# eglrp/fSGM

Hardware: AMD Instinct MI355X
Metric: aggregated cost-volume voxel-paths/s (HxWxDx8 paths), KITTI 1242x375 D=128 (higher is better)
Workload: dtype u8

## Files before the change

### fsgm_amd/csrc/epi_band.hip

```cpp
#include "epi_kernels.h"
#include "fsgm_device.h"
#include "epi_step.h"
#include <type_traits>
#include <stdlib.h>

namespace fsgm {

#ifndef FSGM_BAND_PF
#define FSGM_BAND_PF 2
#endif
#ifndef FSGM_BAND_PF2
#define FSGM_BAND_PF2 1
#endif
#ifndef FSGM_BAND_PF4
#define FSGM_BAND_PF4 3
#endif
#ifndef FSGM_BAND_PFE
#define FSGM_BAND_PFE 4
#endif
#ifndef FSGM_BAND_PFE2
#define FSGM_BAND_PFE2 2
#endif
#ifndef FSGM_BAND_R16
#define FSGM_BAND_R16 1
#endif
#ifndef FSGM_BAND_Y16
#define FSGM_BAND_Y16 0
#endif
#ifndef FSGM_BAND_RECLDS
#define FSGM_BAND_RECLDS 1
#endif
#ifndef FSGM_BAND_SLACK
#define FSGM_BAND_SLACK 32
#endif
#ifndef FSGM_BAND_WAVES
#define FSGM_BAND_WAVES 8
#endif
#ifndef FSGM_BAND_MINW
#define FSGM_BAND_MINW 4
#endif

__device__ __forceinline__ uint32_t pack_hi_bits(const uint32_t (&R)[8]) {
    constexpr uint32_t SEL_HI = 0x07030501u;
    const uint32_t h0 = __builtin_amdgcn_perm(R[1], R[0], SEL_HI), h1 = __builtin_amdgcn_perm(R[3], R[2], SEL_HI);
    const uint32_t h2 = __builtin_amdgcn_perm(R[5], R[4], SEL_HI), h3 = __builtin_amdgcn_perm(R[7], R[6], SEL_HI);
    return h0 | (h1 << 1) | (h2 << 2) | (h3 << 3);
}
__device__ __forceinline__ void unpack_p9(const uint4 v, const uint32_t bits, uint32_t (&R)[8]) {
    const uint32_t w[4] = {v.x, v.y, v.z, v.w};
#pragma unroll
    for (int k = 0; k < 4; k++) {
        const uint32_t hk = (bits >> k) & 0x01010101u;
        R[2 * k] = __builtin_amdgcn_perm(hk, w[k], 0x06020400u);
        R[2 * k + 1] = __builtin_amdgcn_perm(hk, w[k], 0x07030501u);
    }
}

__device__ __forceinline__ void band_unpack_c(const uint4 w, uint32_t (&C)[8]) {
    C[0] = __builtin_amdgcn_perm(w.z, w.x, 0x0C040C00u);
    C[1] = __builtin_amdgcn_perm(w.z, w.x, 0x0C050C01u);
    C[2] = __builtin_amdgcn_perm(w.z, w.x, 0x0C060C02u);
    C[3] = __builtin_amdgcn_perm(w.z, w.x, 0x0C070C03u);
    C[4] = __builtin_amdgcn_perm(w.w, w.y, 0x0C040C00u);
    C[5] = __builtin_amdgcn_perm(w.w, w.y, 0x0C050C01u);
    C[6] = __builtin_amdgcn_perm(w.w, w.y, 0x0C060C02u);
    C[7] = __builtin_amdgcn_perm(w.w, w.y, 0x0C070C03u);
}
template <int LPP, bool MASKED, bool OUT_N>
__device__ __forceinline__ void step_x(uint32_t (&S)[8], const uint32_t (&C)[8], uint32_t (&O)[8], const uint32_t P1pk,
                                       const uint32_t P2pk, const uint32_t kx, const uint32_t K0, const LaneSel sel,
                                       const bool start) {
    uint32_t N[8], YB[8];
    const uint32_t LT = __builtin_amdgcn_perm(S[7], (uint32_t)__builtin_amdgcn_mov_dpp((int)S[7], DPP_ROW_SHR1, 0xF, 0xF, true), sel.lo);
    const uint32_t RT = __builtin_amdgcn_perm((uint32_t)__builtin_amdgcn_mov_dpp((int)S[0], DPP_ROW_SHL1, 0xF, 0xF, true), S[0], sel.hi);
#pragma unroll
    for (int i = 0; i < 8; i++) {
        YB[i] = pk_max3(S[i] + P1pk, i ? S[i - 1] : LT, i < 7 ? S[i + 1] : RT);
        asm("v_xad_u32 %0, %1, %2, %3" : "=v"(N[i]) : "v"(YB[i]), "s"(kx), "v"(C[i]));
    }
    const uint32_t mm = pk_min(pk_min3(N[0], N[1], N[2]), pk_min3(N[3], N[4], pk_min3(N[5], N[6], N[7])));
    uint32_t mx = group_min_u32<LPP>(min_halves(mm));
    if (MASKED && start) mx = K0;
    const uint32_t p2m = __umul24(mx, 0x10001u) + P2pk;
#pragma unroll
    for (int i = 0; i < 8; i++) {
        S[i] = pk_subs(p2m, N[i]);
        O[i] = OUT_N ? N[i] : YB[i];
    }
}

template <int LPP, int NT>
__device__ __forceinline__ uint2 band_nb_entry(const uint32_t d) {
    constexpr uint32_t D = LPP * 16;
    const uint32_t lo = d > 0 ? srow_index<NT>(0, d - 1) * 2u : 0u, hi = d + 1 < D ? srow_index<NT>(0, d + 1) * 2u : 0u;
    return make_uint2(lo | (hi << 16), (d > 0 ? 0x0000FFFFu : 0u) | (d + 1 < D ? 0xFFFF0000u : 0u));
}
template <uint32_t X>
__device__ __forceinline__ uint32_t sconst() { uint32_t r; asm("s_mov_b32 %0, %1" : "=s"(r) : "i"(X)); return r; }

template <int LPP, int NT, bool STAGE>
__device__ __forceinline__ void band_wta_record(const uint32_t (&ST)[8], uint32_t* sRow, const uint2* sNb, int tid, int j,
                                                bool ok, uint8_t* recb, uint8_t* s0b, uint32_t pix,
                                                uint2* stg_rec, uint16_t* stg_s0) {
    srow_store<NT>(sRow, tid, ST);
    const uint32_t IDX[8] = {sconst<0x80000u>(), sconst<0x90001u>(), sconst<0xA0002u>(), sconst<0xB0003u>(),
                             sconst<0xC0004u>(), sconst<0xD0005u>(), sconst<0xE0006u>(), sconst<0xF0007u>()};
    uint32_t K[8];
#pragma unroll
    for (int i = 0; i < 8; i++) K[i] = (ST[i] << 4) | IDX[i];
    const uint32_t kmin = pk_min(pk_min3(K[0], K[1], K[2]), pk_min3(K[3], K[4], pk_min3(K[5], K[6], K[7])));
    const uint32_t k16 = min_halves(kmin);
    uint32_t key;
    asm("v_lshl_or_b32 %0, %1, 4, %2" : "=v"(key) : "v"(k16 & ~15u), "v"((k16 & 15u) | ((uint32_t)j << 4)));
    key = group_min_u32<LPP>(key);
    __builtin_amdgcn_wave_barrier();
    if (j == 0 && ok) {
        const uint2 nb = sNb[key & 0xFFu];
        const uint8_t* row = (const uint8_t*)sRow + tid * 16;
        u16x2 c;
        c[0] = *(const uint16_t*)(row + (nb.x & 0xFFFFu));
        c[1] = *(const uint16_t*)(row + (nb.x >> 16));
        const uint2 rec = make_uint2(__builtin_amdgcn_perm(0u, key, sconst<0x02010C00u>()),
                                     __builtin_bit_cast(uint32_t, c) & nb.y);
        if (STAGE) {
            *stg_rec = rec;
            *stg_s0 = (uint16_t)ST[0];
        } else {
            *(uint2*)(recb + pix * 8u) = rec;
            *(uint16_t*)(s0b + pix * 2u) = (uint16_t)ST[0];
        }
    }
}

template <int LPP, int MODE, int NWV, int PATHS, bool BITS, bool TAP, bool CHAIN>
__global__ __launch_bounds__(NWV * 64, FSGM_BAND_MINW) void band_kernel(BandArgs a) {
    constexpr bool UP = MODE != 0;
    constexpr bool P8 = PATHS == 8;
    constexpr int PXG = 64 / LPP;
    constexpr int R = NWV * PXG;
    constexpr int D = LPP * 16;
    constexpr int SKEW = P8 ? 2 : 1;
    constexpr int NST = P8 ? 3 : 1;
    constexpr int PF = P8 ? (MODE == 2 ? FSGM_BAND_PF2 : FSGM_BAND_PF) : FSGM_BAND_PF4;
    constexpr bool R16 = P8 && MODE == 0 && !CHAIN && FSGM_BAND_R16 != 0;
    constexpr int NSL = R16 ? 2 : NST;
    __shared__ uint2 sNb[MODE == 2 ? D : 1];
    __shared__ uint4 sR16[R16 ? 2 : 1][2][R16 ? (R + 1) * LPP : 1];
    __shared__ uint4 sSt[2][NSL][(R + 1) * LPP];
    __shared__ __attribute__((aligned(16))) uint32_t sRow[MODE == 2 ? NWV * 64 * 8 : 4];
    constexpr bool RECLDS = MODE == 2 && FSGM_BAND_RECLDS != 0 && LPP == 8;
    __shared__ uint2 sRec[RECLDS ? NWV * 64 : 1];
    __shared__ uint16_t sRs0[RECLDS ? NWV * 64 : 1];
    __shared__ uint32_t sTicket;

    const int tid = threadIdx.x, lane = tid & 63, wave = tid >> 6;
    const int g = lane / LPP, j = lane % LPP;
    const int r = wave * PXG + g;
    const int W = a.W, H = a.H, NP = W * H;
    int cband = 0;
    size_t f = blockIdx.x;
    if (CHAIN) {
        if (tid == 0) sTicket = atomicAdd(a.ticket, 1u);
        __syncthreads();
        const uint32_t t = __builtin_amdgcn_readfirstlane(sTicket);
        const uint32_t per = (uint32_t)a.group * (uint32_t)a.nbands, grp = t / per, rem = t - grp * per;
        const uint32_t fin = min((uint32_t)a.group, (uint32_t)a.frames - grp * (uint32_t)a.group);
        cband = (int)(rem / fin);
        f = (size_t)grp * a.group + rem % fin;
        if (cband >= a.nbands || f >= (size_t)a.frames) return;
    }
    constexpr uint32_t VB = (uint32_t)(SKEW * R + PF) * D;
    constexpr bool Y16 = BITS && FSGM_BAND_Y16 != 0;
    const uint8_t* __restrict__ Cf = a.C + f * a.c_frame_stride - VB;
    uint8_t* __restrict__ Yf = a.Y + f * a.y_frame_stride - VB;
    uint8_t* __restrict__ Bf = BITS ? (uint8_t*)(a.Yb + f * a.yb_frame_stride) - (Y16 ? VB : VB / 4) : nullptr;
    uint8_t* __restrict__ Ef = (uint8_t*)(a.edge + f * a.edge_frame_stride);
    const uint32_t tag = CHAIN ? a.tag : 0u;
    uint8_t* __restrict__ recb = MODE == 2 ? (uint8_t*)(a.rec + f * (size_t)NP) : nullptr;
    uint8_t* __restrict__ s0b = MODE == 2 ? (uint8_t*)(a.s0 + f * (size_t)NP) : nullptr;
    const uint32_t P1pk = (uint32_t)a.P1 * 0x10001u, P2 = (uint32_t)a.P2, P2pk = P2 * 0x10001u;
    const uint32_t KX = sconst<0x007F007Fu>(), K0 = 127u - (P2 + (uint32_t)a.P1);
    const uint32_t K1pk = (uint32_t)(PATHS * (a.P1 + a.P2) - (PATHS / 2) * 127) * 0x10001u;
    const uint4 startP = make_uint4(P2 * 0x01010101u, P2 * 0x01010101u, P2 * 0x01010101u, P2 * 0x01010101u);
    const uint32_t DS = sconst<(uint32_t)D>();
    const LaneSel sel = lane_sel<LPP>(j);
    const int elane = min(lane, NST * LPP - 1);

    if (MODE == 2 && tid < D) sNb[tid] = band_nb_entry<LPP, NWV * 64>((uint32_t)tid);

    auto pix_of = [&](int x, int y) -> int { const int p = y * W + x; return UP ? NP - 1 - p : p; };

    for (int yb = CHAIN ? cband * R : 0; yb < (CHAIN ? cband * R + 1 : H); yb += R) {
        const int Rp = min(R, H - yb);
        const int y = yb + r, yc = min(y, H - 1);
        const bool row_ok = r < Rp;
        const int nsteps = W + SKEW * (Rp - 1);
        const bool have_above = yb > 0, last_band = yb + R >= H;
        const bool loader = wave == 0 && lane < NST * LPP && have_above;
        const int r_lo = wave * PXG, r_hi = r_lo + PXG - 1;
        const int act_lo = SKEW * r_lo - (P8 ? 1 : 0), act_hi = W - 1 + SKEW * r_hi;
        const bool wave_rows = r_lo < Rp;
        const int pl_lo = SKEW * r_hi + 1, pl_hi = W - 2 + SKEW * r_lo;
        const bool wave_plain_rows = r_hi < Rp && yb + r_lo >= 1;

        auto vox_lin = [&](int x) -> uint32_t { return (uint32_t)pix_of(x, yc) * D + ((uint32_t)j * 16 + VB); };
        auto vox_off = [&](int u) -> uint32_t { return vox_lin(min(max(u - SKEW * r, 0), W - 1)); };
        uint32_t vpf = vox_lin(PF - 1 - SKEW * r);
        const uint32_t v_lo = vox_lin(UP ? W - 1 : 0), v_hi = vox_lin(UP ? 0 : W - 1);
        const uint32_t emap = (uint32_t)W * (NST * LPP) * 16u;
        const uint8_t* __restrict__ Ein = CHAIN ? Ef + (uint32_t)max(cband - 1, 0) * emap : Ef;
        uint8_t* __restrict__ Eout = CHAIN ? Ef + (uint32_t)cband * emap : Ef;
        auto edge_at = [&](int x) -> const uint8_t* { return Ein + ((uint32_t)min(max(x, 0), W - 1) * (NST * LPP) + (uint32_t)elane) * 16u; };
        bool gave_up = false;
        auto put_above = [&](const int par, const uint4 v) {
            if (R16 && elane / LPP == 2) {
                uint32_t S[8];
                unpack_p(v, S);
                sR16[par][0][elane % LPP] = make_uint4(S[0], S[1], S[2], S[3]);
                sR16[par][1][elane % LPP] = make_uint4(S[4], S[5], S[6], S[7]);
            } else {
                sSt[par][elane / LPP][elane % LPP] = v;
            }
        };
        auto fresh = [&](const uint4 v) -> bool { return (((v.x ^ tag) | (v.y ^ tag) | (v.z ^ tag) | (v.w ^ tag)) & 0x80808080u) == 0u; };
        auto eload = [&](const uint8_t* q) -> uint4 { return CHAIN ? edge_load((const uint4*)q) : load_nt(q); };
        auto settle = [&](uint4 v, const uint8_t* q, const bool mine) -> uint4 {
            if (CHAIN) {
                for (uint32_t spins = 0; !gave_up && !__all(!mine || fresh(v)); spins++) {
                    __builtin_amdgcn_s_sleep(8);
                    if (mine) v = edge_load((const uint4*)q);
                    if (spins > (1u << 18) || ((spins & 1023u) == 1023u && __hip_atomic_load(a.err, __ATOMIC_RELAXED, __HIP_MEMORY_SCOPE_AGENT) != 0u)) {
                        if (lane == 0) atomicOr(a.err, 1u);
                        gave_up = true;
                    }
                }
                v.x &= 0x7F7F7F7Fu; v.y &= 0x7F7F7F7Fu; v.z &= 0x7F7F7F7Fu; v.w &= 0x7F7F7F7Fu;
            }
            return v;
        };

        uint32_t FS[8];
#pragma unroll
        for (int i = 0; i < 8; i++) FS[i] = P2pk;
        uint4 hU = startP, hDp[2] = {startP, startP};
        if (P8 && have_above && wave == 0) {
            const bool mine = r == 0;
            const uint8_t* q0 = Ein + (uint32_t)(0 * LPP + j) * 16u;
            const uint8_t* q1 = Ein + (uint32_t)(1 * LPP + j) * 16u;
            const uint4 v0 = settle(mine ? eload(q0) : startP, q0, mine), v1 = settle(mine ? eload(q1) : startP, q1, mine);
            if (mine) { hU = v0; hDp[1] = v1; }
        }
        if (CHAIN && wave == 0 && have_above) {
            const uint8_t* q = edge_at(min(SKEW + FSGM_BAND_SLACK, W - 1));
            (void)settle(loader ? eload(q) : startP, q, loader);
        }
        if (wave == 0 && have_above) {
            const uint8_t* q = edge_at(SKEW - 1);
            const uint4 v = settle(loader ? eload(q) : startP, q, loader);
            if (loader) put_above(1, v);
        }
        constexpr int NR = MODE == 2 && P8 ? PF + 1 : PF;
        constexpr int UN = P8 && (NR & 1) ? 2 * NR : NR;
        uint4 ringC[NR], ringY[MODE == 2 ? NR : 1];
        constexpr int PFE = CHAIN ? (MODE == 2 ? FSGM_BAND_PFE2 : FSGM_BAND_PFE) : 1;
        uint4 ringE[PFE];
#pragma unroll
        for (int i = 0; i < PFE; i++) ringE[i] = startP;
        uint32_t ringB[MODE == 2 && BITS && !Y16 ? NR : 1];
        uint4 ringB4[MODE == 2 && Y16 ? NR : 1];
#pragma unroll
        for (int i = 0; i < PF; i++) {
            const uint32_t off = vox_off(i);
            ringC[i] = *(const uint4*)(Cf + off);
            if (MODE == 2) {
                ringY[i] = vol_load(Yf + off);
                if (Y16) ringB4[i] = vol_load(Bf + off);
                else if (BITS) ringB[i] = *(const uint32_t*)(Bf + (off >> 2));
            }
        }
        if (loader) {
#pragma unroll
            for (int i = 0; i < PFE; i++) ringE[i] = eload(edge_at(SKEW + i));
        }
        if constexpr (RECLDS) sRec[wave * 64 + lane] = make_uint2(0xFFFFFFFFu, 0xFFFFFFFFu);
        __syncthreads();

        auto do_step = [&](const int u, const int hp, const uint4 cw, const uint4 cy, const uint32_t cb, const uint4 cb4, auto edge_tag) {
            constexpr bool EDGE = decltype(edge_tag)::value;
            const int par = u & 1;
            const int x = u - SKEW * r;
            const bool inside = !EDGE || (row_ok && x >= 0 && x < W);
            const int xc = EDGE ? min(max(x, 0), W - 1) : x;
            uint4 nNow, nLo, nHi;
            if constexpr (R16) { nLo = sR16[par ^ 1][0][r * LPP + j]; nHi = sR16[par ^ 1][1][r * LPP + j]; }
            else nNow = sSt[par ^ 1][P8 ? 2 : 0][r * LPP + j];
            uint32_t CP[8], Y[8], YS[8], S[8];
            band_unpack_c(cw, CP);
            const bool top = EDGE && y == 0;
            {
                const bool st = EDGE && x <= 0;
                if (st) {
#pragma unroll
                    for (int i = 0; i < 8; i++) FS[i] = P2pk;
                }
                step_x<LPP, EDGE, MODE == 2>(FS, CP, YS, P1pk, P2pk, KX, K0, sel, st);
            }
            if (MODE == 2) {
                uint32_t E2[8];
                if (Y16) { E2[0] = cy.x; E2[1] = cy.y; E2[2] = cy.z; E2[3] = cy.w; E2[4] = cb4.x; E2[5] = cb4.y; E2[6] = cb4.z; E2[7] = cb4.w; }
                else if (BITS) unpack_p9(cy, cb, E2);
                else unpack_p(cy, E2);
#pragma unroll
                for (int i = 0; i < 8; i++) YS[i] -= E2[i];
            }
            __builtin_amdgcn_sched_barrier(0);
            uint4 newU, newD, newR;
            {
                unpack_p(P8 ? hU : nNow, S);
                if (top) {
#pragma unroll
                    for (int i = 0; i < 8; i++) S[i] = P2pk;
                }
                step_x<LPP, EDGE, MODE == 2>(S, CP, Y, P1pk, P2pk, KX, K0, sel, top);
                newU = pack_p(S);
                sSt[par][0][(r + 1) * LPP + j] = newU;
#pragma unroll
                for (int i = 0; i < 8; i++) YS[i] += MODE == 2 ? Y[i] + K1pk : Y[i];
            }
            __builtin_amdgcn_sched_barrier(0);
            if constexpr (P8) {
                {
                    const bool st = top || (EDGE && x <= 0);
                    unpack_p(hDp[hp], S);
                    if (st) {
#pragma unroll
                        for (int i = 0; i < 8; i++) S[i] = P2pk;
                    }
                    step_x<LPP, EDGE, MODE == 2>(S, CP, Y, P1pk, P2pk, KX, K0, sel, st);
                    newD = pack_p(S);
                    sSt[par][1][(r + 1) * LPP + j] = newD;
#pragma unroll
                    for (int i = 0; i < 8; i++) YS[i] += Y[i];
                    hDp[hp] = sSt[par ^ 1][1][r * LPP + j];
                    hU = sSt[par ^ 1][0][r * LPP + j];
                }
                __builtin_amdgcn_sched_barrier(0);
                {
                    const bool st = top || (EDGE && x >= W - 1);
                    if (R16) { S[0] = nLo.x; S[1] = nLo.y; S[2] = nLo.z; S[3] = nLo.w; S[4] = nHi.x; S[5] = nHi.y; S[6] = nHi.z; S[7] = nHi.w; }
                    else unpack_p(nNow, S);
                    if (st) {
#pragma unroll
                        for (int i = 0; i < 8; i++) S[i] = P2pk;
                    }
                    step_x<LPP, EDGE, MODE == 2>(S, CP, Y, P1pk, P2pk, KX, K0, sel, st);
                    if constexpr (R16) {
                        sR16[par][0][(r + 1) * LPP + j] = make_uint4(S[0], S[1], S[2], S[3]);
                        sR16[par][1][(r + 1) * LPP + j] = make_uint4(S[4], S[5], S[6], S[7]);
                        if (!last_band && r == R - 1) newR = pack_p(S);
                    } else {
                        newR = pack_p(S);
                        sSt[par][2][(r + 1) * LPP + j] = newR;
                    }
#pragma unroll
                    for (int i = 0; i < 8; i++) YS[i] += Y[i];
                }
            }
            if (!last_band && r == R - 1 && inside) {
                uint8_t* o = Eout + ((uint32_t)xc * (NST * LPP) + (uint32_t)j) * 16u;
                if (CHAIN) {
                    edge_store((uint4*)o, make_uint4(newU.x | tag, newU.y | tag, newU.z | tag, newU.w | tag));
                    if constexpr (P8) {
                        edge_store((uint4*)(o + LPP * 16), make_uint4(newD.x | tag, newD.y | tag, newD.z | tag, newD.w | tag));
                        edge_store((uint4*)(o + 2 * LPP * 16), make_uint4(newR.x | tag, newR.y | tag, newR.z | tag, newR.w | tag));
                    }
                } else {
                    *(uint4*)o = newU;
                    if constexpr (P8) { *(uint4*)(o + LPP * 16) = newD; *(uint4*)(o + 2 * LPP * 16) = newR; }
                }
            }
            if (MODE != 2) {
                if (inside) {
                    const uint32_t so = EDGE ? vox_lin(xc) : vpf;
                    constexpr int SB = EDGE ? 0 : PF * D;
                    if (Y16) {
                        vol_store(Yf + so - SB, make_uint4(YS[0], YS[1], YS[2], YS[3]));
                        vol_store(Bf + so - SB, make_uint4(YS[4], YS[5], YS[6], YS[7]));
                    } else {
                        vol_store(Yf + so - SB, pack_p(YS));
                        if (BITS) *(uint32_t*)(Bf + (so >> 2) - SB / 4) = pack_hi_bits(YS);
                    }
                }
            } else {
                uint32_t ST[8];
#pragma unroll
                for (int i = 0; i < 8; i++) ST[i] = (CP[i] << (P8 ? 2 : 1)) + YS[i];
                if constexpr (RECLDS)
                    band_wta_record<LPP, NWV * 64, true>(ST, sRow, sNb, tid, j, inside, recb, s0b, 0u, &sRec[wave * 64 + g * 8 + (u & 7)], &sRs0[wave * 64 + g * 8 + (u & 7)]);
                else
                    band_wta_record<LPP, NWV * 64, false>(ST, sRow, sNb, tid, j, inside, recb, s0b, (uint32_t)pix_of(xc, yc), nullptr, nullptr);
                if (TAP && inside) {
                    uint32_t* o = a.Sdbg + (f * (size_t)NP + pix_of(xc, yc)) * D + j * 16;
#pragma unroll
                    for (int i = 0; i < 8; i++) { o[i] = ST[i] & 0xFFFFu; o[i + 8] = ST[i] >> 16; }
                }
            }
        };
        auto flush_records = [&](const int u) {
            if constexpr (RECLDS) {
                __builtin_amdgcn_wave_barrier();
                const int fr = lane >> 3, fs = lane & 7;
                const uint2 rc = sRec[wave * 64 + lane];
                const uint16_t s0v = sRs0[wave * 64 + lane];
                sRec[wave * 64 + lane] = make_uint2(0xFFFFFFFFu, 0xFFFFFFFFu);
                const int uu = (u & ~7) + fs, rr = wave * PXG + fr;
                const int xx = uu - SKEW * rr;
                if (rc.x != 0xFFFFFFFFu) {
                    const uint32_t px = (uint32_t)pix_of(xx, yb + rr);
                    *(uint2*)(recb + px * 8u) = rc;
                    *(uint16_t*)(s0b + px * 2u) = s0v;
                }
                __builtin_amdgcn_wave_barrier();
            }
        };
        auto step = [&](const int u, const int hp, const uint4 cw, const uint4 cy, const uint32_t cb, const uint4 cb4) {
            if (wave == 0 && have_above) {
                const uint4 v = settle(ringE[0], edge_at(u + SKEW), loader);
#pragma unroll
                for (int i = 0; i + 1 < PFE; i++) ringE[i] = ringE[i + 1];
                if (loader) {
                    put_above(u & 1, v);
                    ringE[PFE - 1] = eload(edge_at(u + PFE + SKEW));
                }
            }
            if (wave_rows && u >= act_lo && u <= act_hi) {
                if (wave_plain_rows && u >= pl_lo && u <= pl_hi) do_step(u, hp, cw, cy, cb, cb4, std::false_type{});
                else do_step(u, hp, cw, cy, cb, cb4, std::true_type{});
            }
            if constexpr (RECLDS) {
                if ((u & 7) == 7) flush_records(u);
            }
#ifndef FSGM_BAND_NOBAR
            __syncthreads();
#endif
        };

        auto ring_step = [&](const int u, const int i) {
            const int k = i % NR, kl = (i + PF) % NR;
            const uint4 cw = ringC[k];
            const uint4 cy = ringY[MODE == 2 ? k : 0];
            const uint32_t cb = ringB[MODE == 2 && BITS && !Y16 ? k : 0];
            const uint4 cb4 = ringB4[MODE == 2 && Y16 ? k : 0];
            vpf = UP ? vpf - DS : vpf + DS;
            asm("" : "+v"(vpf));
            uint32_t off;
            asm("v_med3_u32 %0, %1, %2, %3" : "=v"(off) : "v"(vpf), "v"(v_lo), "v"(v_hi));
            ringC[kl] = *(const uint4*)(Cf + off);
            if (MODE == 2) {
                ringY[kl] = vol_load(Yf + off);
                if (Y16) ringB4[kl] = vol_load(Bf + off);
                else if (BITS) ringB[kl] = *(const uint32_t*)(Bf + (off >> 2));
            }
            step(u, i & 1, cw, cy, cb, cb4);
        };
        int u0 = 0;
        for (; u0 + UN <= nsteps; u0 += UN) {
#pragma unroll
            for (int i = 0; i < UN; i++) ring_step(u0 + i, i);
        }
#pragma unroll
        for (int i = 0; i < UN - 1; i++)
            if (u0 + i < nsteps) ring_step(u0 + i, i);
        if constexpr (RECLDS) {
            if ((nsteps & 7) != 0) flush_records(nsteps - 1);
        }
        if (!CHAIN) {
            asm volatile("s_waitcnt vmcnt(0)" ::: "memory");
            __syncthreads();
        }
    }
}

size_t band_edge_uint4s(int W, int D, int paths) { const int lpp = agg_packed_lpp(D); return (size_t)W * (paths == 8 ? 3 : 1) * lpp; }
size_t band_bits_u32s(int W, int H, int D) { return (size_t)W * H * agg_packed_lpp(D) * (FSGM_BAND_Y16 ? 4 : 1); }
bool band_needs_bits(int paths, int P1, int P2) { return paths == 8 && 4 * (P1 + P2) > 255; }
bool band_ok(int D, int paths, int P1, int P2, int cmax) {
    return agg_packed_lpp(D) != 0 && P1 >= 0 && P2 >= 0 && P1 + P2 <= 127 && (paths == 8 || paths == 4) && 16 * paths * (cmax + P2 + P1) + 15 < 0x7C00;
}

template <int LPP, int MODE>
static void launch_band_t(hipStream_t st, const BandArgs& a, int frames, int paths) {
    constexpr int NWV = FSGM_BAND_WAVES;
    const bool bits = band_needs_bits(paths, a.P1, a.P2);
    dim3 grid((unsigned)(a.chain ? frames * a.nbands : frames)), block(NWV * 64);
    if (MODE == 2 && a.Sdbg) {
        if (paths == 4)  hipLaunchKernelGGL((band_kernel<LPP, MODE, NWV, 4, false, MODE == 2, false>), grid, block, 0, st, a);
        else if (!bits)  hipLaunchKernelGGL((band_kernel<LPP, MODE, NWV, 8, false, MODE == 2, false>), grid, block, 0, st, a);
        else             hipLaunchKernelGGL((band_kernel<LPP, MODE, NWV, 8, true, MODE == 2, false>), grid, block, 0, st, a);
        return;
    }
    if (a.chain) {
        if (paths == 4)  hipLaunchKernelGGL((band_kernel<LPP, MODE, NWV, 4, false, false, true>), grid, block, 0, st, a);
        else if (!bits)  hipLaunchKernelGGL((band_kernel<LPP, MODE, NWV, 8, false, false, true>), grid, block, 0, st, a);
        else             hipLaunchKernelGGL((band_kernel<LPP, MODE, NWV, 8, true, false, true>), grid, block, 0, st, a);
        return;
    }
    if (paths == 4)  hipLaunchKernelGGL((band_kernel<LPP, MODE, NWV, 4, false, false, false>), grid, block, 0, st, a);
    else if (!bits)  hipLaunchKernelGGL((band_kernel<LPP, MODE, NWV, 8, false, false, false>), grid, block, 0, st, a);
    else             hipLaunchKernelGGL((band_kernel<LPP, MODE, NWV, 8, true, false, false>), grid, block, 0, st, a);
}

int band_rows(int D) { const int lpp = agg_packed_lpp(D); return lpp ? FSGM_BAND_WAVES * (64 / lpp) : 0; }

void launch_band(hipStream_t st, const BandArgs& a, int frames, int paths, int mode) {
#define FSGM_BAND(L) do { if (mode == 0) launch_band_t<L, 0>(st, a, frames, paths); else launch_band_t<L, 2>(st, a, frames, paths); } while (0)
    switch (agg_packed_lpp(a.D)) {
        case 1: FSGM_BAND(1); break;
        case 2: FSGM_BAND(2); break;
        case 4: FSGM_BAND(4); break;
        case 8: FSGM_BAND(8); break;
        case 16: FSGM_BAND(16); break;
        default: break;
    }
#undef FSGM_BAND
}

}
```

Before: 6088 billion.

## Restructure R16 unpacked row-state LDS buffer to single array with per-wave spill slots

Replaces the double-buffered (parity-indexed) unpacked 16-bit row-state LDS arrays with a single buffer plus extra per-wave boundary slots, so intra-wave neighbours read and write in place and only wave-boundary rows use separate slots selected by half-phase. The goal is to cut LDS footprint and index arithmetic, and to defer pack_p of the boundary state to the edge-store path. It also adds an optional R16F switch (off by default) to allow the unpacked path in MODE 2, and uses asm barriers to pin scheduling. The in-place scheme depends on the ordering the half-phase logic provides, which brings a risk of read/write hazards.

```diff
diff --git a/fsgm_amd/csrc/epi_band.hip b/fsgm_amd/csrc/epi_band.hip
--- a/fsgm_amd/csrc/epi_band.hip
+++ b/fsgm_amd/csrc/epi_band.hip
@@ -23,6 +23,9 @@
 #endif
 #ifndef FSGM_BAND_R16
 #define FSGM_BAND_R16 1
+#endif
+#ifndef FSGM_BAND_R16F
+#define FSGM_BAND_R16F 0
 #endif
 #ifndef FSGM_BAND_Y16
 #define FSGM_BAND_Y16 0
@@ -142,10 +145,11 @@
     constexpr int SKEW = P8 ? 2 : 1;
     constexpr int NST = P8 ? 3 : 1;
     constexpr int PF = P8 ? (MODE == 2 ? FSGM_BAND_PF2 : FSGM_BAND_PF) : FSGM_BAND_PF4;
-    constexpr bool R16 = P8 && MODE == 0 && !CHAIN && FSGM_BAND_R16 != 0;
+    constexpr bool R16 = P8 && !CHAIN && (MODE == 2 ? FSGM_BAND_R16F : FSGM_BAND_R16) != 0;
     constexpr int NSL = R16 ? 2 : NST;
+    constexpr int R16N = (R + 1) * LPP, R16X = (NWV + 1) * LPP;
     __shared__ uint2 sNb[MODE == 2 ? D : 1];
-    __shared__ uint4 sR16[R16 ? 2 : 1][2][R16 ? (R + 1) * LPP : 1];
+    __shared__ uint4 sR16[2][R16 ? R16N + R16X : 1];
     __shared__ uint4 sSt[2][NSL][(R + 1) * LPP];
     __shared__ __attribute__((aligned(16))) uint32_t sRow[MODE == 2 ? NWV * 64 * 8 : 4];
     constexpr bool RECLDS = MODE == 2 && FSGM_BAND_RECLDS != 0 && LPP == 8;
@@ -185,6 +189,8 @@
     const uint32_t DS = sconst<(uint32_t)D>();
     const LaneSel sel = lane_sel<LPP>(j);
     const int elane = min(lane, NST * LPP - 1);
+    const int r16rd = g == 0 ? R16N + wave * LPP + j : r * LPP + j;
+    const int r16wr = g == PXG - 1 ? R16N + (wave + 1) * LPP + j : (r + 1) * LPP + j;
 
     if (MODE == 2 && tid < D) sNb[tid] = band_nb_entry<LPP, NWV * 64>((uint32_t)tid);
 
@@ -215,9 +221,13 @@
         auto put_above = [&](const int par, const uint4 v) {
             if (R16 && elane / LPP == 2) {
                 uint32_t S[8];
-                unpack_p(v, S);
-                sR16[par][0][elane % LPP] = make_uint4(S[0], S[1], S[2], S[3]);
-                sR16[par][1][elane % LPP] = make_uint4(S[4], S[5], S[6], S[7]);
+                uint4 w = v;
+                asm volatile("" : "+v"(w.x), "+v"(w.y), "+v"(w.z), "+v"(w.w));
+                unpack_p(w, S);
+                const int wi = (par ? 0 : R16N) + elane % LPP;
+                sR16[0][wi] = make_uint4(S[0], S[1], S[2], S[3]);
+                sR16[1][wi] = make_uint4(S[4], S[5], S[6], S[7]);
+                asm volatile("");
             } else {
                 sSt[par][elane / LPP][elane % LPP] = v;
             }
@@ -291,9 +301,8 @@
             const int x = u - SKEW * r;
             const bool inside = !EDGE || (row_ok && x >= 0 && x < W);
             const int xc = EDGE ? min(max(x, 0), W - 1) : x;
-            uint4 nNow, nLo, nHi;
-            if constexpr (R16) { nLo = sR16[par ^ 1][0][r * LPP + j]; nHi = sR16[par ^ 1][1][r * LPP + j]; }
-            else nNow = sSt[par ^ 1][P8 ? 2 : 0][r * LPP + j];
+            uint4 nNow;
+            if constexpr (!R16) nNow = sSt[par ^ 1][P8 ? 2 : 0][r * LPP + j];
             uint32_t CP[8], Y[8], YS[8], S[8];
             band_unpack_c(cw, CP);
             const bool top = EDGE && y == 0;
@@ -347,17 +356,20 @@
                 __builtin_amdgcn_sched_barrier(0);
                 {
                     const bool st = top || (EDGE && x >= W - 1);
-                    if (R16) { S[0] = nLo.x; S[1] = nLo.y; S[2] = nLo.z; S[3] = nLo.w; S[4] = nHi.x; S[5] = nHi.y; S[6] = nHi.z; S[7] = nHi.w; }
-                    else unpack_p(nNow, S);
+                    if constexpr (R16) {
+                        const int ri = hp ? r16rd : r * LPP + j;
+                        const uint4 nLo = sR16[0][ri], nHi = sR16[1][ri];
+                        S[0] = nLo.x; S[1] = nLo.y; S[2] = nLo.z; S[3] = nLo.w; S[4] = nHi.x; S[5] = nHi.y; S[6] = nHi.z; S[7] = nHi.w;
+                    } else unpack_p(nNow, S);
                     if (st) {
 #pragma unroll
                         for (int i = 0; i < 8; i++) S[i] = P2pk;
                     }
                     step_x<LPP, EDGE, MODE == 2>(S, CP, Y, P1pk, P2pk, KX, K0, sel, st);
                     if constexpr (R16) {
-                        sR16[par][0][(r + 1) * LPP + j] = make_uint4(S[0], S[1], S[2], S[3]);
-                        sR16[par][1][(r + 1) * LPP + j] = make_uint4(S[4], S[5], S[6], S[7]);
-                        if (!last_band && r == R - 1) newR = pack_p(S);
+                        const int wi = hp ? (r + 1) * LPP + j : r16wr;
+                        sR16[0][wi] = make_uint4(S[0], S[1], S[2], S[3]);
+                        sR16[1][wi] = make_uint4(S[4], S[5], S[6], S[7]);
                     } else {
                         newR = pack_p(S);
                         sSt[par][2][(r + 1) * LPP + j] = newR;
@@ -375,6 +387,7 @@
                         edge_store((uint4*)(o + 2 * LPP * 16), make_uint4(newR.x | tag, newR.y | tag, newR.z | tag, newR.w | tag));
                     }
                 } else {
+                    if constexpr (R16) newR = pack_p(S);
                     *(uint4*)o = newU;
                     if constexpr (P8) { *(uint4*)(o + LPP * 16) = newD; *(uint4*)(o + 2 * LPP * 16) = newR; }
                 }
@@ -429,7 +442,7 @@
 #pragma unroll
                 for (int i = 0; i + 1 < PFE; i++) ringE[i] = ringE[i + 1];
                 if (loader) {
-                    put_above(u & 1, v);
+                    put_above(R16 ? hp : u & 1, v);
                     ringE[PFE - 1] = eload(edge_at(u + PFE + SKEW));
                 }
             }
```

After: 6049 billion. No clear change (-0.6%).
